# avadakadabra0909/geth-sharding

Measured on AMD Instinct MI355X. Metric: ecrecover sigs/sec + Keccak collation GB/s, higher is better.
Workload: dtype u32; 1 GPU; 1M-signature secp256k1 ecrecover + Keccak-256 address derivation per GPU (BASELINE.json configs[1]); signatures_per_gpu=1048576, parallelism=shard-partitioned x1, batches_in_flight=2

## Files before the change

geth-sharding_amd/csrc/ecrecover.hip:

```cpp
#include "opcount.cuh"
#include "recover_dev.cuh"
#include "secp256k1_sign.cuh"

namespace gsv {

__global__ __launch_bounds__(256) __attribute__((amdgpu_waves_per_eu(GSV_ECR_WAVES, GSV_ECR_WAVES))) void k_ecrecover(const uint8_t* __restrict__ msg32,
                                                   const uint8_t* __restrict__ sig65, uint32_t n,
                                                   const uint4* __restrict__ gtab,
                                                   uint8_t* __restrict__ pub65,
                                                   uint8_t* __restrict__ addr20,
                                                   uint8_t* __restrict__ status) {
    GSV_LTAB_DECL;
    uint32_t i = blockIdx.x * blockDim.x + threadIdx.x;
    if (i >= n) return;
    const uint8_t* sg = sig65 + (size_t)i * 65;
    uint32_t msg[8], r[8], s[8];
    load32_be(msg, msg32 + (size_t)i * 32);
    load32_be(r, sg);
    load32_be(s, sg + 32);
    uint32_t recid = sg[64];
    fe qx, qy;
    uint32_t st = recover_core(qx, qy, msg, r, s, recid & 3u, gtab, GSV_LTAB_LANE);
    if (recid >= 4) st = GSV_ST_INVALID_RECID;
    bool ok = st == GSV_ST_OK;
    store_pub_addr(pub65 ? pub65 + (size_t)i * 65 : nullptr, addr20 ? addr20 + (size_t)i * 20 : nullptr,
                   ok, qx, qy);
    status[i] = (uint8_t)st;
}

__global__ __launch_bounds__(256) __attribute__((amdgpu_waves_per_eu(GSV_ECR_WAVES, GSV_ECR_WAVES))) void k_sender(const uint8_t* __restrict__ sighash32,
                                                const uint8_t* __restrict__ r32,
                                                const uint8_t* __restrict__ s32,
                                                const uint64_t* __restrict__ v,
                                                const uint8_t* __restrict__ vbig, uint32_t n,
                                                int homestead, const uint4* __restrict__ gtab,
                                                uint8_t* __restrict__ addr20,
                                                uint8_t* __restrict__ status) {
    GSV_LTAB_DECL;
    uint32_t i = blockIdx.x * blockDim.x + threadIdx.x;
    if (i >= n) return;
    uint32_t msg[8], r[8], s[8];
    load32_be(msg, sighash32 + (size_t)i * 32);
    load32_be(r, r32 + (size_t)i * 32);
    load32_be(s, s32 + (size_t)i * 32);
    uint8_t V = (uint8_t)(v[i] - 27u);
    bool valid = vbig[i] == 0 && v[i] <= 0xFFu;
    sc rs, ss;
#pragma unroll
    for (int k = 0; k < 8; k++) {
        rs.v[k] = r[k];
        ss.v[k] = s[k];
    }
    valid = valid && !sc_is_zero(rs) && !sc_is_zero(ss);
    valid = valid && !(homestead && limbs_lt(HALF_N, s));
    valid = valid && limbs_lt(r, SN) && limbs_lt(s, SN) && (V == 0 || V == 1);
    fe qx, qy;
    uint32_t st = recover_core(qx, qy, msg, r, s, V & 1u, gtab, GSV_LTAB_LANE);
    if (!valid) st = GSV_ST_INVALID_SIG;
    store_pub_addr(nullptr, addr20 + (size_t)i * 20, st == GSV_ST_OK, qx, qy);
    status[i] = (uint8_t)st;
}

__global__ __launch_bounds__(256) __attribute__((amdgpu_waves_per_eu(GSV_ECR_WAVES, GSV_ECR_WAVES))) void k_ecrecover_precompile(
    const uint8_t* __restrict__ in128, uint32_t n, const uint4* __restrict__ gtab, uint8_t* __restrict__ out32,
    uint8_t* __restrict__ ok) {
    GSV_LTAB_DECL;
    uint32_t i = blockIdx.x * blockDim.x + threadIdx.x;
    if (i >= n) return;
    const uint8_t* p = in128 + (size_t)i * 128;
    uint32_t msg[8], r[8], s[8];
    load32_be(msg, p);
    load32_be(r, p + 64);
    load32_be(s, p + 96);
    uint32_t hi = 0;
#pragma unroll
    for (int k = 32; k < 63; k++) hi |= p[k];
    uint8_t V = (uint8_t)(p[63] - 27u);
    sc rs, ss;
#pragma unroll
    for (int k = 0; k < 8; k++) {
        rs.v[k] = r[k];
        ss.v[k] = s[k];
    }
    bool valid = hi == 0 && !sc_is_zero(rs) && !sc_is_zero(ss) && limbs_lt(r, SN) && limbs_lt(s, SN) &&
                 (V == 0 || V == 1);
    fe qx, qy;
    uint32_t st = recover_core(qx, qy, msg, r, s, V & 1u, gtab, GSV_LTAB_LANE);
    bool good = valid && st == GSV_ST_OK;
    uint8_t* o = out32 + (size_t)i * 32;
#pragma unroll
    for (int k = 0; k < 12; k++) o[k] = 0;
    store_pub_addr(nullptr, o + 12, good, qx, qy);
    ok[i] = good ? 1 : 0;
}

GSV_DI void gtab_store(uint4* e, const gej9& acc) {
    fe9 zi, zi2, x, y;
    fe9_inv(zi, acc.z);
    fe9_sqr(zi2, zi);
    fe9_mul(x, acc.x, zi2);
    fe9_mul(zi2, zi2, zi);
    fe9_mul(y, acc.y, zi2);
    fe9_normalize_full(x);
    fe9_normalize_full(y);
    e[0] = make_uint4(x.v[0], x.v[1], x.v[2], x.v[3]);
    e[1] = make_uint4(x.v[4], x.v[5], x.v[6], x.v[7]);
    e[2] = make_uint4(x.v[8], y.v[0], y.v[1], y.v[2]);
    e[3] = make_uint4(y.v[3], y.v[4], y.v[5], y.v[6]);
    e[4] = make_uint4(y.v[7], y.v[8], 0u, 0u);
}

__global__ __launch_bounds__(64) void k_gtable_base(uint4* __restrict__ gtab) {
    uint32_t w = threadIdx.x;
    if (w >= (uint32_t)COMB_WINDOWS) return;
    gej9 acc;
    fe9_from_const(acc.x, GX);
    fe9_from_const(acc.y, GY);
    fe9_set_u32(acc.z, 1);
    for (uint32_t k = 0; k < (uint32_t)COMB_BITS * w; k++) gej9_dbl(acc, acc);
    gtab_store(gtab + ((size_t)w << COMB_BITS) * GTAB_ENTRY_U4, acc);
}

__global__ __launch_bounds__(256) void k_gtable_init(uint4* __restrict__ gtab) {
    size_t id = (size_t)blockIdx.x * blockDim.x + threadIdx.x;
    if (id >= GTAB_ENTRIES) return;
    uint32_t w = (uint32_t)(id >> COMB_BITS), d = (uint32_t)(id & ((1u << COMB_BITS) - 1u));
    if (d == 0) return;
    ge9 B;
    gtab_load(B, gtab + ((size_t)w << COMB_BITS) * GTAB_ENTRY_U4);
    gej9 acc;
    bool inf = true;
    acc.x = B.x;
    acc.y = B.y;
    fe9_set_u32(acc.z, 1);
    for (int b = COMB_BITS - 1; b >= 0; b--) {
        if (!inf) gej9_dbl(acc, acc);
        if ((d >> b) & 1u) gej9_add_ge(acc, inf, acc, B);
    }
    gtab_store(gtab + id * GTAB_ENTRY_U4, acc);
}

__global__ __launch_bounds__(256) void k_synth_sign(uint64_t seed, uint32_t n,
                                                    const uint4* __restrict__ gtab,
                                                    uint8_t* __restrict__ msg32,
                                                    uint8_t* __restrict__ sig65,
                                                    uint8_t* __restrict__ pub65,
                                                    uint8_t* __restrict__ addr20) {
    uint32_t i = blockIdx.x * blockDim.x + threadIdx.x;
    if (i >= n) return;
    sc d, k, m;
    derive32(d.v, seed, i, 0x79656bu);
    derive32(m.v, seed, i, 0x67736du);
    derive32(k.v, seed, i, 0x65636eu);
    uint32_t r[8], s[8], recid;
    fe px, py;
    ecdsa_sign(r, s, recid, px, py, d, k, m.v, gtab);
    uint8_t* sg = sig65 + (size_t)i * 65;
    limbs_to_be(sg, r);
    limbs_to_be(sg + 32, s);
    sg[64] = (uint8_t)recid;
    limbs_to_be(msg32 + (size_t)i * 32, m.v);
    store_pub_addr(pub65 ? pub65 + (size_t)i * 65 : nullptr, addr20 ? addr20 + (size_t)i * 20 : nullptr,
                   true, px, py);
}

hipError_t launch_gtable_init(uint4* gtab, hipStream_t st) {
    hipLaunchKernelGGL(k_gtable_base, dim3(1), dim3(64), 0, st, gtab);
    hipError_t e = hipGetLastError();
    if (e != hipSuccess) return e;
    hipLaunchKernelGGL(k_gtable_init, dim3((unsigned)((GTAB_ENTRIES + 255) / 256)), dim3(256), 0, st, gtab);
    return hipGetLastError();
}

hipError_t launch_ecrecover(const uint8_t* msg32, const uint8_t* sig65, uint32_t n, const uint4* gtab,
                            uint8_t* pub65, uint8_t* addr20, uint8_t* status, hipStream_t st) {
    if (n == 0) return hipSuccess;
    hipLaunchKernelGGL(k_ecrecover, dim3((n + 255) / 256), dim3(256), 0, st, msg32, sig65, n, gtab,
                       pub65, addr20, status);
    return hipGetLastError();
}

hipError_t launch_sender(const uint8_t* sighash32, const uint8_t* r32, const uint8_t* s32,
                         const uint64_t* v, const uint8_t* vbig, uint32_t n, int homestead,
                         const uint4* gtab, uint8_t* addr20, uint8_t* status, hipStream_t st) {
    if (n == 0) return hipSuccess;
    hipLaunchKernelGGL(k_sender, dim3((n + 255) / 256), dim3(256), 0, st, sighash32, r32, s32, v, vbig,
                       n, homestead, gtab, addr20, status);
    return hipGetLastError();
}

hipError_t launch_ecrecover_precompile(const uint8_t* in128, uint32_t n, const uint4* gtab, uint8_t* out32,
                                       uint8_t* ok, hipStream_t st) {
    if (n == 0) return hipSuccess;
    hipLaunchKernelGGL(k_ecrecover_precompile, dim3((n + 255) / 256), dim3(256), 0, st, in128, n, gtab, out32, ok);
    return hipGetLastError();
}

hipError_t launch_synth_sign(uint64_t seed, uint32_t n, const uint4* gtab, uint8_t* msg32,
                             uint8_t* sig65, uint8_t* pub65, uint8_t* addr20, hipStream_t st) {
    if (n == 0) return hipSuccess;
    hipLaunchKernelGGL(k_synth_sign, dim3((n + 255) / 256), dim3(256), 0, st, seed, n, gtab, msg32,
                       sig65, pub65, addr20);
    return hipGetLastError();
}

}

GSV_OPCOUNT_READER(ecrecover)
```

geth-sharding_amd/csrc/gsv_internal.h:

```cpp
#pragma once
#include <hip/hip_runtime.h>
#include <stdint.h>

#include "../../include/gsv.h"
#include "block_header_host.h"

namespace gsv {

hipError_t launch_gtable_init(uint4* gtab, hipStream_t st);
hipError_t launch_ecrecover(const uint8_t* msg32, const uint8_t* sig65, uint32_t n, const uint4* gtab,
                            uint8_t* pub65, uint8_t* addr20, uint8_t* status, hipStream_t st);
hipError_t launch_sender(const uint8_t* sighash32, const uint8_t* r32, const uint8_t* s32,
                         const uint64_t* v, const uint8_t* vbig, uint32_t n, int homestead,
                         const uint4* gtab, uint8_t* addr20, uint8_t* status, hipStream_t st);
hipError_t launch_ecrecover_precompile(const uint8_t* in128, uint32_t n, const uint4* gtab, uint8_t* out32,
                                       uint8_t* ok, hipStream_t st);
hipError_t launch_synth_sign(uint64_t seed, uint32_t n, const uint4* gtab, uint8_t* msg32,
                             uint8_t* sig65, uint8_t* pub65, uint8_t* addr20, hipStream_t st);

hipError_t launch_ecverify(const uint8_t* msg32, const uint8_t* sig64, const uint8_t* pub65, const uint8_t* publen,
                           uint32_t n, const uint4* gtab, uint8_t* ok, hipStream_t st);
hipError_t launch_pubkey_parse(const uint8_t* pub65, const uint8_t* publen, uint32_t n, uint8_t* out65, uint8_t* ok,
                               hipStream_t st);

hipError_t launch_ecsign(const uint8_t* msg32, const uint8_t* seckey32, uint32_t n, const uint4* gtab, uint8_t* sig65,
                         uint8_t* status, hipStream_t st);
hipError_t launch_pubkey_create(const uint8_t* seckey32, uint32_t n, const uint4* gtab, uint8_t* pub65,
                                uint8_t* addr20, uint8_t* status, hipStream_t st);

constexpr uint32_t TXS_SUFFIX_WORDS = 20, TXS_V_WORDS = 17;
struct TxSignSuffix {
    uint32_t w[TXS_SUFFIX_WORDS];
    uint32_t len;
};
struct TxSignVTable {
    uint32_t w[4 * TXS_V_WORDS];
    uint32_t len[4];
};
constexpr size_t TXS_WORK_PER = 16 + 32 + 65 + 1;
hipError_t launch_tx_sighash(const uint8_t* d_rlp, const uint64_t* d_off, uint32_t n, const TxSignSuffix& sfx,
                             uint32_t* d_rec, uint32_t* d_msg32, hipStream_t st);
hipError_t launch_tx_seal(const uint8_t* d_rlp, const uint64_t* d_off, uint32_t n, const TxSignVTable& vt,
                          uint64_t growth, const uint32_t* d_rec, const uint8_t* d_sig65, const uint8_t* d_sign_st,
                          uint8_t* d_out, uint32_t* d_out_len, uint8_t* d_hash32, uint8_t* d_status, hipStream_t st);

hipError_t launch_ecdh(const uint8_t* point64, const uint8_t* scalar32, uint32_t n, uint8_t* xy64, uint8_t* x32,
                       uint8_t* keys48, uint8_t* status, hipStream_t st);

constexpr size_t ECIES_WORK_DEC = 48 + 64 + 1, ECIES_WORK_ENC = 48 + 65 + 1 + 1;
hipError_t launch_ecies_parse(const uint8_t* ct, const uint64_t* ct_off, const uint8_t* seckey32, uint32_t n,
                              uint8_t* point64, uint8_t* status, hipStream_t st);
hipError_t launch_ecies_open(const uint8_t* ct, const uint64_t* ct_off, const uint8_t* s2, const uint64_t* s2_off,
                             uint32_t n, uint8_t* work, uint8_t* msg_out, uint32_t* msg_len, uint8_t* status,
                             hipStream_t st);
hipError_t launch_ecies_seal(const uint8_t* msg, const uint64_t* msg_off, const uint8_t* iv16, const uint8_t* s2,
                             const uint64_t* s2_off, uint32_t n, uint8_t* work, uint8_t* ct_out, uint8_t* status,
                             hipStream_t st);

hipError_t launch_keccak256(const uint8_t* data, const uint64_t* off, uint32_t n, uint8_t* out32,
                            hipStream_t st);

hipError_t launch_sha256(const uint8_t* data, const uint64_t* off, uint32_t n, uint8_t* out32, hipStream_t st);
hipError_t launch_ripemd160(const uint8_t* data, const uint64_t* off, uint32_t n, uint8_t* out32, hipStream_t st);

constexpr int GSV_HOOK_TAIL = -1;

struct TriePlan;
size_t chunk_root_scratch_bytes(const TriePlan* plan, uint32_t nbodies);
hipError_t launch_chunk_root_plan(const TriePlan* plan, const uint8_t* d_bodies, const uint64_t* d_body_off,
                                  uint32_t nbodies, uint8_t* d_scratch, uint8_t* d_roots, hipStream_t st,
                                  void (*timer_begin)(void*, int), void (*timer_end)(void*, int),
                                  void* tctx);

size_t derive_sha_scratch_bytes(const TriePlan* plan, uint32_t nlists);
hipError_t launch_derive_sha_plan(const TriePlan* plan, uint32_t nlists, const uint8_t* d_vals,
                                  const uint64_t* d_voff, uint64_t vend, const uint64_t* d_leaf_base, uint8_t* d_lmsg, uint8_t* d_leafrefs, uint8_t* d_scratch, uint8_t* d_roots,
                                  hipStream_t st, void (*timer_begin)(void*, int), void (*timer_end)(void*, int),
                                  void* tctx);
hipError_t launch_poc_expand(const uint8_t* d_bodies, const uint64_t* d_in_off, const uint64_t* d_out_off,
                             uint32_t nbodies, uint64_t max_out, const uint8_t* d_salt, uint32_t slen, uint8_t* d_out,
                             hipStream_t st);

size_t header_scratch_bytes(uint32_t n);
hipError_t launch_header_verify(const uint8_t* d_sid32, const uint8_t* d_root32, const uint8_t* d_per32,
                                const uint8_t* d_prop20, const uint8_t* d_sig65, const uint8_t* d_nil, uint32_t n,
                                const uint4* gtab, uint8_t* d_scratch, uint8_t* d_hash32, uint8_t* d_signer20,
                                uint8_t* d_status, hipStream_t st);

constexpr int GSV_BN_LAYOUT_FINAL3 = 1, GSV_BN_LAYOUT_MILLER2 = 2, GSV_BN_LAYOUT_MILLERW2 = 8,
              GSV_BN_LAYOUT_LINESW2 = 16, GSV_BN_LAYOUT_MILLERL = 32;
constexpr int BN_FINAL_SLOTS = 8;
hipError_t launch_bn256_pairing(const uint8_t* d_in, const uint64_t* d_pair_src, uint32_t npairs,
                                const uint32_t* d_lane_first, const uint32_t* d_pidx, uint32_t nlanes,
                                const uint32_t* d_check_lane, const uint8_t* d_cbad, uint32_t nchecks,
                                uint8_t* d_pstat, uint32_t* d_lines, uint8_t* d_lstat, uint32_t* d_fv,
                                uint32_t* d_fws, uint32_t maxl, uint8_t* d_verdict, int layout, hipStream_t st, void (*timer_begin)(void*, int),
                                void (*timer_end)(void*, int), void* tctx);
hipError_t launch_bn256_synth(uint64_t seed, uint32_t nchecks, uint8_t* d_out, uint8_t* d_expect, hipStream_t st);

hipError_t launch_bn256_g1_add(const uint8_t* d_in128, uint32_t n, uint8_t* d_out64, uint8_t* d_status,
                               hipStream_t st);
hipError_t launch_bn256_g1_mul(const uint8_t* d_in96, uint32_t n, uint8_t* d_out64, uint8_t* d_status,
                               int bitserial, hipStream_t st);

hipError_t launch_modexp(const uint8_t* d_in, uint32_t n, uint32_t bl, uint32_t el, uint32_t ml, uint8_t* d_out,
                         uint8_t* d_work, hipStream_t st);

hipError_t launch_ethash_items(const uint8_t* d_cache, uint64_t cache_bytes, uint32_t first, uint32_t count,
                               uint8_t* d_out64, hipStream_t st);
hipError_t launch_ethash_light(const uint8_t* d_cache, uint64_t cache_bytes, uint64_t dataset_bytes,
                               const uint8_t* d_hash32, const uint64_t* d_nonce, uint32_t n, uint8_t* d_mix32,
                               uint8_t* d_result32, hipStream_t st);
hipError_t launch_ethash_verify(const uint8_t* d_cache, uint64_t cache_bytes, uint64_t dataset_bytes,
                                const uint8_t* d_hash32, const uint64_t* d_nonce, const uint8_t* d_mix32,
                                const uint8_t* d_difficulty32, uint32_t n, uint8_t* d_status, hipStream_t st);
hipError_t launch_ethash_full(const uint8_t* d_dataset, uint64_t dataset_bytes, const uint8_t* d_hash32,
                              const uint64_t* d_nonce, uint32_t n, uint8_t* d_mix32, uint8_t* d_result32,
                              hipStream_t st);
hipError_t launch_ethash_verify_full(const uint8_t* d_dataset, uint64_t dataset_bytes, const uint8_t* d_hash32,
                                     const uint64_t* d_nonce, const uint8_t* d_mix32, const uint8_t* d_difficulty32,
                                     uint32_t n, uint8_t* d_status, hipStream_t st);
hipError_t launch_ethash_search(const uint8_t* d_dataset, uint64_t dataset_bytes, const uint8_t* d_hash32,
                                const uint8_t* d_difficulty32, const uint64_t* d_start, uint32_t n, uint32_t span,
                                uint32_t* d_offset, hipStream_t st);
hipError_t launch_ethash_finish(const uint8_t* d_dataset, uint64_t dataset_bytes, const uint8_t* d_hash32,
                                const uint64_t* d_start, const uint32_t* d_offset, uint32_t n, uint64_t* d_nonce_out,
                                uint8_t* d_mix32, uint8_t* d_result32, uint8_t* d_found, hipStream_t st);

hipError_t launch_block_header(const uint8_t* d_rlp, const uint64_t* d_off, uint32_t n, const uint8_t* d_parent_rlp,
                               uint32_t parent_len, uint8_t* d_work, uint8_t* d_hash32, uint8_t* d_hnn32,
                               uint64_t* d_nonce, uint8_t* d_mix32, uint8_t* d_difficulty32, uint64_t* d_number,
                               uint8_t* d_status, hipStream_t st);
hipError_t launch_block_header_rules(uint8_t* d_work, uint32_t n, const bh::Config& cfg, uint64_t now, uint8_t* d_pre,
                                     uint8_t* d_post, uint8_t* d_want32, hipStream_t st);
hipError_t launch_block_header_merge(const uint8_t* d_pre, const uint8_t* d_seal, const uint8_t* d_seals,
                                     const uint8_t* d_post, uint32_t n, uint8_t* d_status, hipStream_t st);
hipError_t launch_calc_difficulty(uint8_t* d_work, uint32_t n, const bh::Config& cfg, const uint64_t* d_time,
                                  uint8_t* d_want32, uint8_t* d_status, hipStream_t st);

hipError_t launch_receipt_scan(const uint8_t* d_vals, const uint64_t* d_voff, uint32_t n, const uint64_t* d_list_off,
                               uint32_t n_lists, uint64_t vals_bytes, uint8_t* d_work, uint8_t* d_receipt_status,
                               hipStream_t st);
hipError_t launch_receipt_bloom(const uint8_t* d_vals, const uint64_t* d_voff, uint32_t n, uint64_t vals_bytes,
                                const uint8_t* d_work, uint8_t* d_list_bloom, uint8_t* d_receipt_bloom,
                                hipStream_t st);
hipError_t launch_receipt_lists(const uint64_t* d_list_off, uint32_t n_lists, uint32_t n, uint64_t vals_bytes,
                                const uint8_t* d_work, const uint8_t* d_receipt_status, uint8_t* d_list_bloom,
                                uint64_t* d_gas_used, uint8_t* d_list_status, hipStream_t st);
hipError_t launch_receipt_check(const uint8_t* d_list_status, uint32_t n_lists, const uint8_t* d_list_bloom,
                                uint8_t* d_root32, const uint64_t* d_gas_used, const uint8_t* d_want_bloom,
                                const uint8_t* d_want_root32, const uint64_t* d_want_gas, uint8_t* d_status,
                                hipStream_t st);
hipError_t launch_bloom9(const uint8_t* d_data, const uint64_t* d_off, uint32_t n, uint16_t* d_idx, hipStream_t st);

hipError_t launch_header_hash_unsigned(const uint8_t* d_sid32, const uint8_t* d_root32, const uint8_t* d_per32,
                                       const uint8_t* d_prop20, uint32_t n, uint8_t* d_hash32, hipStream_t st);

hipError_t launch_blob_serialize(const uint8_t* d_blobs, uint64_t begin, uint64_t end, const void* d_ents,
                                 const uint32_t* d_chunk_blob, const uint8_t* d_skip_evm, uint64_t nchunks,
                                 uint8_t* d_out, hipStream_t st);
hipError_t launch_blob_strip(const uint8_t* d_bodies, uint64_t begin, uint64_t end, const uint64_t* d_body_off,
                             const uint32_t* d_body_len, const uint64_t* d_data_off, uint32_t n, uint64_t max_region,
                             uint8_t* d_data, hipStream_t st);
hipError_t launch_blob_unpack(const void* d_recs, const uint32_t* d_cnt, uint32_t n, uint32_t max_blobs,
                              uint32_t* d_start, uint32_t* d_len, uint8_t* d_skip, hipStream_t st);
hipError_t launch_proposer_mask(const uint8_t* d_over, uint32_t n, uint8_t* d_root32, uint8_t* d_hash32,
                                uint8_t* d_sig65, uint8_t* d_status, hipStream_t st);

struct BlobRec {
    uint32_t first_chunk;
    uint32_t nchunks;
    uint32_t len;
    uint32_t skip_evm;
};
size_t blob_rec_bytes();
hipError_t launch_partition_pack(const uint8_t* d_root, const uint32_t* d_ntx, const uint8_t* d_bm, uint32_t n,
                                 uint32_t per, uint32_t R, uint32_t bm, int32_t status, uint8_t* d_block,
                                 hipStream_t st);
hipError_t launch_partition_unpack(const uint8_t* d_all, uint32_t nranks, uint32_t n_total, uint32_t R, uint32_t bm,
                                   size_t B, uint8_t* d_root, uint32_t* d_ntx, uint8_t* d_bm, int32_t* d_rank_status,
                                   hipStream_t st);
hipError_t launch_blob_index(const uint8_t* d_bodies, const uint64_t* d_off, const uint32_t* d_len,
                             uint32_t n_shards, uint32_t max_txs, void* d_blobs, uint32_t* d_ntx, hipStream_t st);
hipError_t launch_notary_tx(const uint8_t* d_bodies, const uint64_t* d_off, const void* d_blobs,
                            const uint32_t* d_ntx, uint32_t n_shards, uint32_t max_txs, const uint8_t* d_cid64,
                            const uint8_t* d_suffix, uint32_t slen, int signer_kind, const uint4* gtab,
                            uint8_t* d_bitmap, uint32_t bm_bytes, uint8_t* d_senders, uint8_t* d_status,
                            hipStream_t st);
hipError_t launch_notary_synth(uint64_t seed, uint32_t shard0, uint32_t n_shards, uint32_t txs_per_shard,
                               const uint4* gtab, uint8_t* d_bodies, uint8_t* d_exp_status, uint8_t* d_exp_sender,
                               hipStream_t st);

constexpr int COMB_BITS = 20;
constexpr int COMB_WINDOWS = (256 + COMB_BITS - 1) / COMB_BITS;
static_assert(COMB_BITS >= 4 && COMB_BITS <= 26, "comb window width");
constexpr size_t GTAB_ENTRIES = (size_t)COMB_WINDOWS << COMB_BITS;
constexpr size_t GTAB_ENTRY_BYTES = 80;
constexpr size_t GTAB_BYTES = GTAB_ENTRIES * GTAB_ENTRY_BYTES;

}
```

geth-sharding_amd/csrc/recover_dev.cuh:

```cuda
#pragma once
#include "gsv_internal.h"
#include "secp256k1_glv.cuh"
#include "secp256k1_comb.cuh"
#include "secp256k1_point.cuh"

namespace gsv {


GSV_DI bool recover_tail_twisted(fe& qx, fe& qy, const gej9& p1, bool p1inf, const gej9& p2, bool p2inf,
                                 const fe9& c, uint32_t par) {
    fe9 x3a, db, y3a, y3b, z;
    fe9 s1p, s2;
    bool exc;
    {
        fe9 z1z1, zz, z2z2, u1, h, t;
        fe9_sqr(z1z1, p1.z);
        fe9_sqr(zz, p2.z);
        fe9_mul(z2z2, c, zz);
        fe9_mul(u1, p1.x, z2z2);
        fe9_mul_sub(h, p2.x, z1z1, u1);
        fe9_mul(s1p, p1.y, p2.z);
        fe9_mul(s1p, s1p, z2z2);
        fe9_mul(s2, p2.y, p1.z);
        fe9_mul(s2, s2, z1z1);
        exc = !p1inf && fe9_is_zero_weak(h);
        fe9 hh, hhh, v, cs1, a1;
        fe9_sqr(hh, h);
        fe9_mul(hhh, h, hh);
        fe9_mul(v, u1, hh);
        fe9_mul(cs1, c, s1p);
        fe9_sqr_sub2<2>(a1, s2, hhh, v);
        fe9_mul_add(x3a, cs1, s1p, a1);
        fe9_mul(t, s2, s1p);
        fe9_add(db, t, t);
        fe9 da, ndb, e;
        fe9_sub<1>(da, v, x3a);
        fe9_neg<2>(ndb, db);
        fe9_dot(y3a, s2, da, cs1, ndb);
        fe9_add(e, da, hhh);
        fe9_normalize_weak(e);
        fe9_neg<1>(t, e);
        fe9_dot(y3b, s2, db, s1p, t);
        fe9_mul(t, p1.z, p2.z);
        fe9_mul(z, t, h);
    }
    if (FE9_ANY(exc)) {
        gej9 d;
        gej9_dbl(d, p2);
        fe9_cmov(x3a, d.x, exc);
        fe9_cmov(y3a, d.y, exc);
        fe9_cmov(z, d.z, exc);
        fe9_cmov(db, s1p, exc);
        fe9_cmov(y3b, s2, exc);
    }
    if (FE9_ANY(p1inf)) {
        fe9 zero;
        fe9_set_u32(zero, 0);
        fe9_cmov(x3a, p2.x, p1inf);
        fe9_cmov(y3a, p2.y, p1inf);
        fe9_cmov(z, p2.z, p1inf);
        fe9_cmov(db, zero, p1inf);
        fe9_cmov(y3b, zero, p1inf);
    }
    fe9 m, s0;
    bool ok;
    {
        fe9 z2, t, w;
        fe9_sqr(z2, z);
        fe9_sqr(t, z2);
        fe9_mul(t, t, c);
        fe9_pow_pm3_4(w, t);
        fe9_mul(m, w, z);
        fe9_mul(t, c, m);
        fe9_mul(s0, t, z);
        fe9_sqr(t, s0);
        fe9_normalize_full(t);
        fe9 cc = c;
        fe9_normalize_full(cc);
        ok = fe9_eq_canon(t, cc) && !p2inf;
    }
    fe9 s0n = s0;
    fe9_normalize_full(s0n);
    bool flip = (s0n.v[0] & 1u) != par;
    fe9 pb, qb;
    fe9_mul(pb, s0, db);
    fe9_mul(qb, s0, y3b);
    if (FE9_ANY(exc)) {
        fe9 a, b2;
        fe9_add(a, y3b, pb);
        fe9_sub<1>(b2, y3b, pb);
        fe9_cmov(b2, a, flip);
        bool rr0 = fe9_is_zero(b2);
        ok = ok && !(exc && !rr0);
        fe9 zero;
        fe9_set_u32(zero, 0);
        fe9_cmov(pb, zero, exc);
        fe9_cmov(qb, zero, exc);
    }
    fe9 m2, m3, n, xs, ys;
    fe9_sqr(m2, m);
    fe9_mul(m3, m2, m);
    fe9_neg<1>(n, pb);
    fe9_cmov(n, pb, flip);
    fe9_add(xs, x3a, n);
    fe9_neg<1>(n, y3a);
    fe9_cmov(n, y3a, !flip);
    fe9_add(ys, n, qb);
    fe9 x, y;
    fe9_mul(x, xs, m2);
    fe9_mul(y, ys, m3);
    fe9_normalize_full(x);
    fe9_normalize_full(y);
    fe9_to_words(qx.v, x);
    fe9_to_words(qy.v, y);
    return ok;
}

GSV_DI uint32_t recover_core(fe& qx, fe& qy, const uint32_t msg[8], const uint32_t r[8],
                             const uint32_t s[8], uint32_t recid, const uint4* __restrict__ gtab,
                             uint32_t* __restrict__ ltab) {
    bool ok = limbs_lt(r, SN) && limbs_lt(s, SN);
    sc rs, ss, m;
#pragma unroll
    for (int i = 0; i < 8; i++) {
        rs.v[i] = r[i];
        ss.v[i] = s[i];
    }
    ok = ok && !sc_is_zero(rs) && !sc_is_zero(ss);
    sc_cond_sub_n(m.v, msg, 0);

    fe9 x;
    {
        bool hi = (recid & 2u) != 0;
        ok = ok && (!hi || limbs_lt(r, P_MINUS_N));
        uint32_t xw[8];
        uint64_t c = 0;
#pragma unroll
        for (int i = 0; i < 8; i++) {
            c = (uint64_t)r[i] + (hi ? SN[i] : 0u) + hi32(c);
            xw[i] = lo32(c);
        }
        fe9_from_words(x, xw);
    }
    fe9 y, t;
    fe9 c;
    curve_rhs9(c, x);
    fe9_mul(t, c, x);
    fe9_sqr(y, c);
    x = t;
    sc rn, u1, u2;
    modinv30_words(rn.v, rs.v, MI30_N);
    sc_mul(u1, rn, m);
    sc_neg(u1, u1);
    sc_mul(u2, rn, ss);

    gej9 acc;
    bool ainf;
    glv_mul_point(acc, ainf, u2, x, y, ltab);

    gej9 accg;
    bool ginf;
    comb_mul_g9(accg, ginf, u1, gtab);

    ok = recover_tail_twisted(qx, qy, accg, ginf, acc, ainf, c, recid & 1u) && ok;
    return ok ? GSV_ST_OK : GSV_ST_RECOVER_FAILED;
}

}
```

geth-sharding_amd/csrc/secp256k1_scalar.cuh:

```cuda
#pragma once
#include <hip/hip_runtime.h>
#include <stdint.h>

#define GSV_DI __device__ __forceinline__

#include "mul_asm.cuh"
#include "opcount.cuh"
#include "secp256k1_dev.cuh"

namespace gsv {

struct fe { uint32_t v[8]; };
struct sc { uint32_t v[8]; };

GSV_DI uint32_t lo32(uint64_t x) { return (uint32_t)x; }
GSV_DI uint32_t hi32(uint64_t x) { return (uint32_t)(x >> 32); }
GSV_DI uint32_t addc(uint32_t a, uint32_t b, uint32_t& c) {
    uint32_t co;
    uint32_t r = __builtin_addc(a, b, c, &co);
    c = co;
    return r;
}
GSV_DI uint32_t subb(uint32_t a, uint32_t b, uint32_t& br) {
    uint32_t bo;
    uint32_t r = __builtin_subc(a, b, br, &bo);
    br = bo;
    return r;
}

GSV_DI void limbs_from_be(uint32_t v[8], const uint8_t* b) {
#pragma unroll
    for (int i = 0; i < 8; i++) {
        const uint8_t* p = b + 28 - 4 * i;
        v[i] = ((uint32_t)p[0] << 24) | ((uint32_t)p[1] << 16) | ((uint32_t)p[2] << 8) | p[3];
    }
}
GSV_DI void load32_be(uint32_t v[8], const uint8_t* p) { limbs_from_be(v, p); }
GSV_DI void limbs_to_be(uint8_t* b, const uint32_t v[8]) {
#pragma unroll
    for (int i = 0; i < 8; i++) {
        uint8_t* p = b + 28 - 4 * i;
        p[0] = (uint8_t)(v[i] >> 24);
        p[1] = (uint8_t)(v[i] >> 16);
        p[2] = (uint8_t)(v[i] >> 8);
        p[3] = (uint8_t)v[i];
    }
}

GSV_DI bool limbs_zero(const uint32_t v[8]) {
    uint32_t o = 0;
#pragma unroll
    for (int i = 0; i < 8; i++) o |= v[i];
    return o == 0;
}
GSV_DI bool limbs_lt(const uint32_t x[8], const uint32_t m[8]) {
    uint32_t br = 0;
#pragma unroll
    for (int i = 0; i < 8; i++) (void)subb(x[i], m[i], br);
    return br != 0;
}

GSV_DI void sc_cond_sub_n(uint32_t r[8], const uint32_t x[8], uint32_t extra_carry) {
    uint32_t y[8], c = 0;
#pragma unroll
    for (int i = 0; i < 8; i++) y[i] = addc(x[i], i < 5 ? SNC[i] : 0u, c);
    uint32_t ge = c | extra_carry;
#pragma unroll
    for (int i = 0; i < 8; i++) r[i] = ge ? y[i] : x[i];
}

GSV_DI void sc_reduce(sc& r, const uint32_t t[16]) {
    const uint32_t C4[4] = {SNC[0], SNC[1], SNC[2], SNC[3]};
    uint32_t p[12], m[13], c = 0;
    mul_8x4_fx(p, t + 8, C4);
#pragma unroll
    for (int i = 0; i < 8; i++) m[i] = addc(t[i], p[i], c);
#pragma unroll
    for (int i = 8; i < 12; i++) m[i] = addc(p[i], 0u, c);
    m[12] = c;
    c = 0;
#pragma unroll
    for (int i = 4; i < 12; i++) m[i] = addc(m[i], t[4 + i], c);
    m[12] += c;
    uint32_t p2[9], m2[10];
    mul_5x4_fx(p2, m + 8, C4);
    c = 0;
#pragma unroll
    for (int i = 0; i < 8; i++) m2[i] = addc(m[i], p2[i], c);
    m2[8] = addc(p2[8], 0u, c);
    m2[9] = c;
    c = 0;
#pragma unroll
    for (int i = 4; i < 9; i++) m2[i] = addc(m2[i], m[4 + i], c);
    m2[9] += c;
    uint32_t p3[6], m3[8];
    mul_2x4_fx(p3, m2 + 8, C4);
    c = 0;
#pragma unroll
    for (int i = 0; i < 6; i++) m3[i] = addc(m2[i], p3[i], c);
    m3[6] = addc(m2[6], 0u, c);
    m3[7] = addc(m2[7], 0u, c);
    uint32_t c2 = 0;
    m3[4] = addc(m3[4], m2[8], c2);
    m3[5] = addc(m3[5], m2[9], c2);
    m3[6] = addc(m3[6], 0u, c2);
    m3[7] = addc(m3[7], 0u, c2);
    sc_cond_sub_n(r.v, m3, c | c2);
}

GSV_DI void sc_mul(sc& r, const sc& a, const sc& b) {
    GSV_OPC(OPC_SC_MUL);
    uint32_t t[16];
    mul_8x8_fx(t, a.v, b.v);
    sc_reduce(r, t);
}
GSV_DI bool sc_is_zero(const sc& a) { return limbs_zero(a.v); }
GSV_DI void sc_neg(sc& r, const sc& a) {
    bool z = sc_is_zero(a);
    int64_t br = 0;
#pragma unroll
    for (int i = 0; i < 8; i++) {
        int64_t t = (int64_t)SN[i] - a.v[i] + br;
        r.v[i] = z ? 0u : (uint32_t)t;
        br = t >> 32;
    }
}
GSV_DI void sc_add(sc& r, const sc& a, const sc& b) {
    uint32_t s[8], c = 0;
#pragma unroll
    for (int i = 0; i < 8; i++) s[i] = addc(a.v[i], b.v[i], c);
    sc_cond_sub_n(r.v, s, c);
}

GSV_DI void sc_from_const(sc& r, const uint32_t c[8]) {
#pragma unroll
    for (int i = 0; i < 8; i++) r.v[i] = c[i];
}
GSV_DI bool sc_is_high(const sc& a) { return limbs_lt(HALF_N, a.v); }

GSV_DI bool seckey_ok(const sc& d) { return limbs_lt(d.v, SN) && !sc_is_zero(d); }
GSV_DI void sc_set_one_unless(sc& k, bool ok) {
#pragma unroll
    for (int j = 0; j < 8; j++) k.v[j] = ok ? k.v[j] : (j == 0 ? 1u : 0u);
}

}
```

Baseline: 126.4 million sigs/s.

## Batch r^-1 scalar inversions with Montgomery trick in a pre-pass kernel

Adds a pre-pass kernel that computes modular inverses of r for groups of RINV_K signatures per lane using Montgomery's batch inversion trick, staging prefix products and results in the pub65 output buffer. The main ecrecover kernel then loads r^-1 from that buffer instead of running a per-signature modinv30. This trades one inversion per signature for roughly three scalar multiplications plus one inversion per group, at the cost of an extra kernel launch and strided unaligned global memory traffic. It only applies when pub65 is requested; otherwise the old path runs.

```diff
diff --git a/geth-sharding_amd/csrc/ecrecover.hip b/geth-sharding_amd/csrc/ecrecover.hip
--- a/geth-sharding_amd/csrc/ecrecover.hip
+++ b/geth-sharding_amd/csrc/ecrecover.hip
@@ -1,13 +1,56 @@
 #include "opcount.cuh"
 #include "recover_dev.cuh"
+#include "secp256k1_rinv.cuh"
 #include "secp256k1_sign.cuh"
 
 namespace gsv {
 
+struct RinvRows {
+    const uint8_t* sig;
+    uint8_t* pub;
+    static constexpr size_t STEP = 64 * 65;
+    GSV_DI void get(uint32_t i, sc& x) const {
+        const uint8_t* p = sig + i * STEP;
+#pragma unroll
+        for (int k = 0; k < 8; k++) x.v[k] = ld32u(p + 4 * k);
+    }
+    GSV_DI void value(sc& x) const {
+#pragma unroll
+        for (int k = 0; k < 4; k++) {
+            uint32_t lo = __builtin_bswap32(x.v[7 - k]), hi = __builtin_bswap32(x.v[k]);
+            x.v[k] = lo;
+            x.v[7 - k] = hi;
+        }
+    }
+    GSV_DI void put(uint32_t i, const sc& x) const {
+#pragma unroll
+        for (int k = 0; k < 8; k++) st32u(pub + i * STEP + 4 * k, x.v[k]);
+    }
+    GSV_DI void take(uint32_t i, sc& x) const {
+#pragma unroll
+        for (int k = 0; k < 8; k++) x.v[k] = ld32u(pub + i * STEP + 4 * k);
+    }
+};
+
+__global__ __launch_bounds__(64) void k_rinv_batch(const uint8_t* __restrict__ sig65, uint32_t n,
+                                                   uint8_t* __restrict__ pub65) {
+    size_t first = (size_t)blockIdx.x * (64 * RINV_K) + threadIdx.x;
+    if (first >= n) return;
+    size_t left = (n - first + 63) / 64;
+    RinvRows rows{sig65 + first * 65, pub65 + first * 65};
+    sc_batch_inverse(rows, left < (size_t)RINV_K ? (uint32_t)left : (uint32_t)RINV_K);
+}
+
+template <bool RINV_GIVEN>
+struct PubRows { typedef uint8_t* __restrict__ type; };
+template <>
+struct PubRows<true> { typedef uint8_t* type; };
+
+template <bool RINV_GIVEN>
 __global__ __launch_bounds__(256) __attribute__((amdgpu_waves_per_eu(GSV_ECR_WAVES, GSV_ECR_WAVES))) void k_ecrecover(const uint8_t* __restrict__ msg32,
                                                    const uint8_t* __restrict__ sig65, uint32_t n,
                                                    const uint4* __restrict__ gtab,
-                                                   uint8_t* __restrict__ pub65,
+                                                   typename PubRows<RINV_GIVEN>::type pub65,
                                                    uint8_t* __restrict__ addr20,
                                                    uint8_t* __restrict__ status) {
     GSV_LTAB_DECL;
@@ -20,7 +63,8 @@
     load32_be(s, sg + 32);
     uint32_t recid = sg[64];
     fe qx, qy;
-    uint32_t st = recover_core(qx, qy, msg, r, s, recid & 3u, gtab, GSV_LTAB_LANE);
+    uint32_t st = recover_core<RINV_GIVEN>(qx, qy, msg, r, s, recid & 3u, gtab, GSV_LTAB_LANE,
+                                           RINV_GIVEN ? pub65 + (size_t)i * 65 : nullptr);
     if (recid >= 4) st = GSV_ST_INVALID_RECID;
     bool ok = st == GSV_ST_OK;
     store_pub_addr(pub65 ? pub65 + (size_t)i * 65 : nullptr, addr20 ? addr20 + (size_t)i * 20 : nullptr,
@@ -175,7 +219,17 @@
 hipError_t launch_ecrecover(const uint8_t* msg32, const uint8_t* sig65, uint32_t n, const uint4* gtab,
                             uint8_t* pub65, uint8_t* addr20, uint8_t* status, hipStream_t st) {
     if (n == 0) return hipSuccess;
-    hipLaunchKernelGGL(k_ecrecover, dim3((n + 255) / 256), dim3(256), 0, st, msg32, sig65, n, gtab,
+    if (!pub65) {
+        hipLaunchKernelGGL(k_ecrecover<false>, dim3((n + 255) / 256), dim3(256), 0, st, msg32, sig65, n, gtab,
+                           pub65, addr20, status);
+        return hipGetLastError();
+    }
+    constexpr uint32_t PER_WAVE = 64u * RINV_K;
+    hipLaunchKernelGGL(k_rinv_batch, dim3((unsigned)(((uint64_t)n + PER_WAVE - 1) / PER_WAVE)), dim3(64), 0, st,
+                       sig65, n, pub65);
+    hipError_t e = hipGetLastError();
+    if (e != hipSuccess) return e;
+    hipLaunchKernelGGL(k_ecrecover<true>, dim3((n + 255) / 256), dim3(256), 0, st, msg32, sig65, n, gtab,
                        pub65, addr20, status);
     return hipGetLastError();
 }
diff --git a/geth-sharding_amd/csrc/gsv_internal.h b/geth-sharding_amd/csrc/gsv_internal.h
--- a/geth-sharding_amd/csrc/gsv_internal.h
+++ b/geth-sharding_amd/csrc/gsv_internal.h
@@ -198,4 +198,10 @@
 constexpr size_t GTAB_ENTRY_BYTES = 80;
 constexpr size_t GTAB_BYTES = GTAB_ENTRIES * GTAB_ENTRY_BYTES;
 
+#ifndef GSV_RINV_K
+#define GSV_RINV_K 16
+#endif
+constexpr int RINV_K = GSV_RINV_K;
+static_assert(RINV_K >= 1 && RINV_K <= 64, "r values per inversion");
+
 }
diff --git a/geth-sharding_amd/csrc/recover_dev.cuh b/geth-sharding_amd/csrc/recover_dev.cuh
--- a/geth-sharding_amd/csrc/recover_dev.cuh
+++ b/geth-sharding_amd/csrc/recover_dev.cuh
@@ -116,9 +116,10 @@
     return ok;
 }
 
+template <bool RINV_GIVEN = false>
 GSV_DI uint32_t recover_core(fe& qx, fe& qy, const uint32_t msg[8], const uint32_t r[8],
                              const uint32_t s[8], uint32_t recid, const uint4* __restrict__ gtab,
-                             uint32_t* __restrict__ ltab) {
+                             uint32_t* __restrict__ ltab, const uint8_t* rinv = nullptr) {
     bool ok = limbs_lt(r, SN) && limbs_lt(s, SN);
     sc rs, ss, m;
 #pragma unroll
@@ -149,7 +150,12 @@
     fe9_sqr(y, c);
     x = t;
     sc rn, u1, u2;
-    modinv30_words(rn.v, rs.v, MI30_N);
+    if constexpr (RINV_GIVEN) {
+#pragma unroll
+        for (int i = 0; i < 8; i++) rn.v[i] = ld32u(rinv + 4 * i);
+    } else {
+        modinv30_words(rn.v, rs.v, MI30_N);
+    }
     sc_mul(u1, rn, m);
     sc_neg(u1, u1);
     sc_mul(u2, rn, ss);
diff --git a/geth-sharding_amd/csrc/secp256k1_rinv.cuh b/geth-sharding_amd/csrc/secp256k1_rinv.cuh
--- /dev/null
+++ b/geth-sharding_amd/csrc/secp256k1_rinv.cuh
@@ -0,0 +1,112 @@
+#pragma once
+#include <stdint.h>
+
+#include "modinv30.cuh"
+
+#if defined(__HIPCC__)
+#include "secp256k1_scalar.cuh"
+#define RINV_FN __device__ __forceinline__
+#else
+#define RINV_FN static inline
+namespace gsv {
+struct sc { uint32_t v[8]; };
+static constexpr uint32_t SN[8] = {0xD0364141u, 0xBFD25E8Cu, 0xAF48A03Bu, 0xBAAEDCE6u,
+                                   0xFFFFFFFEu, 0xFFFFFFFFu, 0xFFFFFFFFu, 0xFFFFFFFFu};
+static inline void sc_mul(sc& r, const sc& a, const sc& b) {
+    static constexpr uint32_t C[5] = {0x2FC9BEBFu, 0x402DA173u, 0x50B75FC4u, 0x45512319u, 1u};
+    uint32_t t[24] = {0};
+    for (int i = 0; i < 8; i++) {
+        uint64_t c = 0;
+        for (int j = 0; j < 8; j++) {
+            c += (uint64_t)a.v[i] * b.v[j] + t[i + j];
+            t[i + j] = (uint32_t)c;
+            c >>= 32;
+        }
+        t[i + 8] = (uint32_t)c;
+    }
+    for (;;) {
+        bool hi = false;
+        for (int i = 8; i < 24; i++) hi = hi || t[i] != 0;
+        if (!hi) break;
+        uint32_t h[16], u[24] = {0};
+        for (int i = 0; i < 16; i++) h[i] = t[8 + i];
+        for (int i = 0; i < 8; i++) u[i] = t[i];
+        for (int i = 0; i < 16; i++) {
+            uint64_t c = 0;
+            for (int j = 0; j < 5 && i + j < 24; j++) {
+                c += (uint64_t)h[i] * C[j] + u[i + j];
+                u[i + j] = (uint32_t)c;
+                c >>= 32;
+            }
+            for (int k = i + 5; c != 0 && k < 24; k++) {
+                c += u[k];
+                u[k] = (uint32_t)c;
+                c >>= 32;
+            }
+        }
+        for (int i = 0; i < 24; i++) t[i] = u[i];
+    }
+    int64_t br = 0;
+    uint32_t d[8];
+    for (int i = 0; i < 8; i++) {
+        int64_t x = (int64_t)t[i] - SN[i] + br;
+        d[i] = (uint32_t)x;
+        br = x >> 32;
+    }
+    for (int i = 0; i < 8; i++) r.v[i] = br ? t[i] : d[i];
+}
+}
+#endif
+
+namespace gsv {
+
+RINV_FN void sc_rinv_operand(sc& x) {
+    uint32_t nz = 0;
+    int64_t br = 0;
+#pragma unroll
+    for (int i = 0; i < 8; i++) {
+        nz |= x.v[i];
+        br = ((int64_t)x.v[i] - (int64_t)SN[i] + br) >> 32;
+    }
+    bool ok = nz != 0 && br != 0;
+#pragma unroll
+    for (int i = 0; i < 8; i++) x.v[i] = ok ? x.v[i] : (i == 0 ? 1u : 0u);
+}
+
+template <class Slots>
+RINV_FN void sc_batch_inverse(Slots& sl, uint32_t cnt) {
+    sc acc, x;
+    sl.get(0, acc);
+    sl.value(acc);
+    sc_rinv_operand(acc);
+    if (cnt > 1) sl.get(1, x);
+    for (uint32_t i = 1; i < cnt; i++) {
+        sc nx = x;
+        sl.put(i, acc);
+        if (i + 1 < cnt) sl.get(i + 1, nx);
+        sl.value(x);
+        sc_rinv_operand(x);
+        sc_mul(acc, acc, x);
+        x = nx;
+    }
+    sc inv, p = acc;
+    if (cnt > 1) sl.take(cnt - 1, p);
+    modinv30_words(inv.v, acc.v, MI30_N);
+    for (uint32_t i = cnt - 1; i >= 1; i--) {
+        sc np = p, nx = x;
+        if (i > 1) {
+            sl.take(i - 1, np);
+            sl.get(i - 1, nx);
+        }
+        sl.value(x);
+        sc_rinv_operand(x);
+        sc_mul(p, p, inv);
+        sl.put(i, p);
+        sc_mul(inv, inv, x);
+        p = np;
+        x = nx;
+    }
+    sl.put(0, inv);
+}
+
+}
diff --git a/geth-sharding_amd/csrc/secp256k1_scalar.cuh b/geth-sharding_amd/csrc/secp256k1_scalar.cuh
--- a/geth-sharding_amd/csrc/secp256k1_scalar.cuh
+++ b/geth-sharding_amd/csrc/secp256k1_scalar.cuh
@@ -46,6 +46,13 @@
         p[3] = (uint8_t)v[i];
     }
 }
+
+GSV_DI uint32_t ld32u(const uint8_t* p) {
+    uint32_t w;
+    __builtin_memcpy(&w, p, 4);
+    return w;
+}
+GSV_DI void st32u(uint8_t* p, uint32_t w) { __builtin_memcpy(p, &w, 4); }
 
 GSV_DI bool limbs_zero(const uint32_t v[8]) {
     uint32_t o = 0;
```

New measurement: 129.3 million sigs/s, median of 6. +2.3%, better.
